# amoretti86/PSVO

Measured on AMD Instinct MI355X. Metric: particle-steps/sec, higher is better.
Workload: dtype f32

## Files before the change

psvo_amd/csrc/bsim_bwd2_impl.h:

```cpp
#pragma once
#define PSVO_BSIM_BWD_V2_UNIT 1
#include "bsim_bwd_impl.h"

namespace psvo {
PSVO_TIMERS_DEFINE(bsim_bwd2)

#define PSVO_GARG(args_type, field) ::psvo::as_global(PSVO_ARG(args_type, field))

__device__ __forceinline__ float swap_add32(float lo, float hi) {
    asm volatile("s_nop 1\n\tv_permlane32_swap_b32 %0, %1" : "+v"(lo), "+v"(hi));
    return lo + hi;
}
__device__ __forceinline__ float swap_add16(float lo, float hi) {
    asm volatile("s_nop 1\n\tv_permlane16_swap_b32 %0, %1" : "+v"(lo), "+v"(hi));
    return lo + hi;
}
__device__ __forceinline__ float row_sum16(float v) {
    v += dpp_mov<0x128, 0xF, 0xF, true>(v, v);
    v += dpp_mov<0x124, 0xF, 0xF, true>(v, v);
    v += dpp_mov<0x122, 0xF, 0xF, true>(v, v);
    v += dpp_mov<0x121, 0xF, 0xF, true>(v, v);
    return v;
}

__device__ __forceinline__ float rs_bit3(float lo, float hi) {
    float r;
    asm volatile("s_nop 1\n\t"
                 "v_add_f32_dpp %0, %1, %1 row_ror:8 row_mask:0xf bank_mask:0x3\n\t"
                 "v_add_f32_dpp %0, %2, %2 row_ror:8 row_mask:0xf bank_mask:0xc"
                 : "=&v"(r) : "v"(lo), "v"(hi));
    return r;
}
__device__ __forceinline__ float rs_bit2(float lo, float hi) {
    float r;
    asm volatile("s_nop 1\n\t"
                 "v_add_f32_dpp %0, %1, %1 row_shl:4 row_mask:0xf bank_mask:0x5\n\t"
                 "v_add_f32_dpp %0, %2, %2 row_shr:4 row_mask:0xf bank_mask:0xa"
                 : "=&v"(r) : "v"(lo), "v"(hi));
    return r;
}
template <int K>
__device__ __forceinline__ void row_reduce_scatter(const float (&v)[4 * K], float (&out)[K]) {
    float h[2 * K];
#pragma unroll
    for (int i = 0; i < 2 * K; ++i) h[i] = rs_bit3(v[i], v[2 * K + i]);
#pragma unroll
    for (int i = 0; i < K; ++i) out[i] = group_sum<4>(rs_bit2(h[i], h[K + i]));
}

typedef float f4v __attribute__((ext_vector_type(4)));
typedef __bf16 bf8v __attribute__((ext_vector_type(8)));

__device__ __forceinline__ void bf16_split3(float v, unsigned& h, unsigned& m, unsigned& l) {
    const unsigned hb = __float_as_uint(v) & 0xffff0000u;
    const float r = v - __uint_as_float(hb);
    const unsigned mb = __float_as_uint(r) & 0xffff0000u;
    const float r2 = r - __uint_as_float(mb);
    h = hb >> 16;
    m = mb >> 16;
    l = __float_as_uint(r2) >> 16;
}
__device__ __forceinline__ uint4 bf16x3_a(float v) {
    unsigned h, m, l;
    bf16_split3(v, h, m, l);
    return make_uint4(h | (h << 16), m | (h << 16), l | (m << 16), m | (l << 16));
}
__device__ __forceinline__ uint4 bf16x3_b(float v) {
    unsigned h, m, l;
    bf16_split3(v, h, m, l);
    return make_uint4(h | (m << 16), h | (l << 16), h | (m << 16), l | (m << 16));
}

template <int DX, int DY, int H, int M, int JM>
__global__ void __launch_bounds__(256, 2) bsim_bwd2_kernel(const BsimBwdArgs a) {
    using MQ = MlpLds<DX, H, DX, 1>;
    using MG = MlpLds<DX, H, DY, 1>;
    using AC = BAcc<DX>;
    constexpr int kN = AC::kSg + DY;
    constexpr int PS = (JM == 3) ? 20 : (DX == 4 && JM == 0) ? 5 : BTileSlot<DX>::kFloats;
    constexpr int FO = (JM == 3) ? 16 : 0;
    constexpr int NA = DX + 1;
    constexpr int PART = 2;
    constexpr int G = M * PART;
    constexpr int CPW = 64 / G;
    constexpr int CM = CPW * M;
    constexpr int NF = DX + 2;
    constexpr int UVS = (2 * DX + 3) & ~3;
    constexpr int JC = (JM == 0 && DX == 4) ? 2 : (JM || DX >= 3) ? 4 : 8;
    constexpr bool RO = (DX == 4) && (JM == 0);
    constexpr bool kSplitTile = (DX == 4) && (JM == 0);
    static_assert(CM == 32 && (M % 4) == 0, "two lanes per (chain, m): M in {4, 8, 16, 32}");
    extern __shared__ __attribute__((aligned(16))) float smem[];

    const int tid = threadIdx.x, lane = tid & 63, wave = tid >> 6;
    constexpr int NTB = 256, nwv = 4;
    const int B = a.B, T = a.T, N = a.N;
    const int NP = ((N + 127) / 128) * 128;
    const int nch = NP / (16 * JC);
    const int b = blockIdx.y, blk = blockIdx.x, nblk = gridDim.x;
    constexpr int cpb = nwv * CPW;
    const int cl = lane / G, part = (lane / M) & 1, m = lane % M;
    const bool h0 = (part == 0);
    const int n_raw = blk * cpb + wave * CPW + cl;
    const bool valid = n_raw < N;
    const int n = valid ? n_raw : N - 1;
    const bool srow = valid && h0;
    const bool lead = srow && (m == 0);
    const int j16 = lane & 15, g = lane >> 4;

    float* wf = smem;
    float* wg = wf + MQ::kSize;
    float* wqi = wg + MG::kSize;
    float* tile = wqi + MQ::kSize;
    float* jacc = tile + 2 * NP * PS;
    float* xch = jacc + nwv * NA * NP;
    float* uvx = xch + nwv * NF * CM;
    float* red = uvx + nwv * CM * UVS;
    float* const xw = xch + wave * NF * CM;
    float* const uw = uvx + wave * CM * UVS;
    float* const ja = jacc + wave * NA * NP;

    MQ::load(wf, a.f, tid, NTB);
    MG::load(wg, a.g, tid, NTB);
    MQ::load(wqi, a.q1inv, tid, NTB);

    const float kappa = sqrtf(0.5f * kLog2e);
    float isf[DX], rp[DX], isfk[DX], isg[DY];
#pragma unroll
    for (int d = 0; d < DX; ++d) {
        isf[d] = 1.f / a.sig_f[d];
        rp[d] = isf[d] * kappa;
        isfk[d] = isf[d] / kappa;
    }
    float ikap2 = 1.f / (kappa * kappa);
#pragma unroll
    for (int e = 0; e < DY; ++e) isg[e] = 1.f / a.sig_g[e];
    float pc[DX], pic[DX], pi1[DX], pi2[DX];
#pragma unroll
    for (int d = 0; d < DX; ++d) {
        pi1[d] = 1.f / a.sig_q1inv[d];
        pi2[d] = 1.f / a.sig_bq2[d];
        pic[d] = pi1[d] + pi2[d];
        pc[d] = 1.f / pic[d];
    }
    float s_init[DX], is_init[DX], i_isig[DX], im[DX], mi[DX];
#pragma unroll
    for (int d = 0; d < DX; ++d) {
        s_init[d] = a.sig_init[d];
        is_init[d] = 1.f / s_init[d];
        i_isig[d] = 1.f / a.isig[d];
        im[d] = a.imean[b * DX + d];
        mi[d] = a.minit[b * DX + d];
    }
    if constexpr (DX <= 2) {
        keep_in_vgpr(isf); keep_in_vgpr(rp); keep_in_vgpr(isfk); keep_in_vgpr(isg); keep_in_vgpr(ikap2);
        keep_in_vgpr(pc); keep_in_vgpr(pic); keep_in_vgpr(pi1); keep_in_vgpr(pi2);
    }
    const float ninf = -__builtin_huge_valf();
    const float aw = valid ? as_global(a.dscore)[(size_t)b * N + n] : 0.f;

    const unsigned NM = (unsigned)N * M;
    unsigned o_nm = 4u * ((unsigned)b * NM + n * M + m);
    unsigned o_dnm[DX], o_knm[DY], o_dn[DX];
#pragma unroll
    for (int d = 0; d < DX; ++d) {
        o_dnm[d] = 4u * (((unsigned)b * DX + d) * NM + n * M + m);
        o_dn[d] = 4u * (((unsigned)b * DX + d) * N + n);
    }
#pragma unroll
    for (int k = 0; k < DY; ++k) o_knm[k] = 4u * (((unsigned)b * DY + k) * NM + n * M + m);
    unsigned o_n = 4u * ((unsigned)b * N + n);
    unsigned o_d = 4u * ((unsigned)b * DX), o_k = 4u * ((unsigned)b * DY);
    const unsigned s_nm = 4u * B * NM, s_dnm = s_nm * DX, s_knm = s_nm * DY, s_dn = 4u * B * DX * N, s_n = 4u * B * N,
                   s_d = 4u * B * DX, s_k = 4u * B * DY;

    float st[DX + 1], st_l = 0.f;
    int st_t = 0;
    auto put_slot = [&](float* buf, int j, const float (&raw)[DX + 1], float l) {
        float F[DX];
#pragma unroll
        for (int d = 0; d < DX; ++d) F[d] = raw[d] * rp[d];
        const float W = j < N ? (raw[DX] - l) * kLog2e : ninf;
        if constexpr (JM == 3) {
            const float Wf = fmaxf(W, -1e30f);
            uint4* q = reinterpret_cast<uint4*>(buf + j * PS);
            q[0] = bf16x3_b(F[0]);
            q[1] = bf16x3_b(F[DX > 1 ? 1 : 0]);
            q[2] = bf16x3_b(Wf - (F[0] * F[0] + F[DX > 1 ? 1 : 0] * F[DX > 1 ? 1 : 0]));
            q[3] = bf16x3_b(1.f);
            *reinterpret_cast<float4*>(buf + j * PS + 16) = make_float4(F[0], F[DX > 1 ? 1 : 0], 0.f, 0.f);
        } else if constexpr (JM == 2) {
            *reinterpret_cast<float4*>(buf + j * PS) = make_float4(F[0], F[1], W - (F[0] * F[0] + F[DX > 1 ? 1 : 0] * F[DX > 1 ? 1 : 0]), 1.f);
        } else if constexpr (DX <= 3) {
            float4 v;
            v.x = F[0];
            v.y = DX > 1 ? F[DX > 1 ? 1 : 0] : 0.f;
            v.z = DX > 2 ? F[DX > 2 ? 2 : 0] : 0.f;
            v.w = W;
            *reinterpret_cast<float4*>(buf + j * PS) = v;
        } else if constexpr (kSplitTile) {
            *reinterpret_cast<float4*>(buf + 4 * j) = make_float4(F[0], F[1], F[2], F[3]);
            buf[4 * NP + j] = W;
        } else {
            *reinterpret_cast<float4*>(buf + j * PS) = make_float4(F[0], F[1], F[2], F[3]);
            *reinterpret_cast<float4*>(buf + j * PS + 4) = make_float4(W, 0.f, 0.f, 0.f);
        }
    };
    auto tile_entry = [&](const float* buf, int j, float (&F)[DX], float& W) {
        if constexpr (kSplitTile) {
            const float4 e = *reinterpret_cast<const float4*>(buf + 4 * j);
            F[0] = e.x; F[DX > 1 ? 1 : 0] = e.y; F[DX > 2 ? 2 : 0] = e.z; F[DX > 3 ? 3 : 0] = e.w;
            W = buf[4 * NP + j];
        } else {
            read_slot<DX>(buf + j * PS, F, W);
        }
    };
    static_assert(offsetof(BsimBwdArgs, logW) - offsetof(BsimBwdArgs, Fm) == 8 &&
                  offsetof(BsimBwdArgs, lse) - offsetof(BsimBwdArgs, Fm) == 16 && offsetof(BsimBwdArgs, Fm) % 32 == 0,
                  "BsimBwdArgs: forward-tile pointer block");
    auto get_slot = [&](int tt, int j, float (&raw)[DX + 1], gptr<const float> Fm, gptr<const float> logW) {
        const unsigned tb = (unsigned)tt * B + b;
        const unsigned jc = j < N ? j : N - 1;
#pragma unroll
        for (int d = 0; d < DX; ++d) raw[d] = ldf(Fm, 4u * ((tb * DX + d) * N + jc));
        raw[DX] = ldf(logW, 4u * (tb * N + jc));
    };
    float st2[DX + 1];
    const bool two_slots = (DX >= 3) && NP > NTB;
    auto stage_load = [&](int tt) {
        unsigned long long pt[4];
        arg_block<4>((unsigned)offsetof(BsimBwdArgs, Fm), pt);
        st_t = tt;
        const gptr<const float> p_Fm = as_global<const float>(pt[0]), p_logW = as_global<const float>(pt[1]);
        st_l = ldf(as_global<const float>(pt[2]), 4u * ((unsigned)tt * B + b));
        if (tid < NP) get_slot(tt, tid, st, p_Fm, p_logW);
        if (two_slots && tid + NTB < NP) get_slot(tt, tid + NTB, st2, p_Fm, p_logW);
    };
    auto stage_store = [&](float* buf) {
        if (tid < NP) put_slot(buf, tid, st, st_l);
        if (two_slots && tid + NTB < NP) put_slot(buf, tid + NTB, st2, st_l);
        for (int j = tid + (two_slots ? 2 : 1) * NTB; j < NP; j += NTB) {
            float raw[DX + 1];
            get_slot(st_t, j, raw, PSVO_GARG(BsimBwdArgs, Fm), PSVO_GARG(BsimBwdArgs, logW));
            put_slot(buf, j, raw, st_l);
        }
    };
    if (T >= 2) {
        stage_load(0);
        stage_store(tile);
    }
    __syncthreads();

    constexpr bool kAccLds = (DX >= 3);
    constexpr int kRowsA = 2 * DX + DY, kRowsB = 5 * DX, kSlotsB = 8;
    float acc[kAccLds ? 1 : kN];
    float* const accA = red + 16 + wave * (kRowsA * 32 + kRowsB * kSlotsB);
    float* const accB = accA + kRowsA * 32;
    auto acc_is_lead = [](int k) { return k < 4 * DX || (k >= 5 * DX && k < 6 * DX); };
    auto acc_row = [](int k) {
        return k < 4 * DX ? k : k < 5 * DX ? k - 4 * DX : k < 6 * DX ? 4 * DX + (k - 5 * DX)
               : k < 7 * DX ? DX + (k - 6 * DX) : 2 * DX + (k - 7 * DX);
    };
    const int s32 = cl * M + m;
    if constexpr (kAccLds) {
        for (int i = lane; i < kRowsA * 32 + kRowsB * kSlotsB; i += 64) accA[i] = 0.f;
    } else {
#pragma unroll
        for (int i = 0; i < kN; ++i) acc[i] = 0.f;
    }
    auto acc_add = [&](int k, float v) {
        if constexpr (kAccLds) {
            if (acc_is_lead(k)) atomicAdd(&accB[acc_row(k) * kSlotsB + cl], v);
            else atomicAdd(&accA[acc_row(k) * 32 + s32], v);
        } else {
            acc[k] += v;
        }
    };
    float dX[DX];
#pragma unroll
    for (int d = 0; d < DX; ++d) dX[d] = 0.f;

    struct StepIn {
        float eps[DX], bm[DX], xp[DX], mu1[DX], y[DY], om, lam2;
        int sel;
    };
    static_assert(offsetof(BsimBwdArgs, dscore) - offsetof(BsimBwdArgs, obs) == 56 && offsetof(BsimBwdArgs, obs) % 64 == 0 &&
                  offsetof(BsimBwdArgs, eps_b) - offsetof(BsimBwdArgs, obs) == 8 &&
                  offsetof(BsimBwdArgs, bwX) - offsetof(BsimBwdArgs, obs) == 16 &&
                  offsetof(BsimBwdArgs, sel) - offsetof(BsimBwdArgs, obs) == 24 &&
                  offsetof(BsimBwdArgs, lam2_all) - offsetof(BsimBwdArgs, obs) == 32 &&
                  offsetof(BsimBwdArgs, om_all) - offsetof(BsimBwdArgs, obs) == 40 &&
                  offsetof(BsimBwdArgs, mu1_all) - offsetof(BsimBwdArgs, obs) == 48, "BsimBwdArgs: input pointer block");
    auto load_step = [&](bool lst, bool fst, StepIn& s) {
        unsigned long long pb[8];
        arg_block<8>((unsigned)offsetof(BsimBwdArgs, obs), pb);
        const gptr<const float> p_obs = as_global<const float>(pb[0]);
        const gptr<const float> p_eps = as_global<const float>(pb[1]);
        const gptr<const float> p_bwX = as_global<const float>(pb[2]);
        const gptr<const int32_t> p_sel = as_global<const int32_t>(pb[3]);
        const gptr<const float> p_lam2 = as_global<const float>(pb[4]);
        const gptr<const float> p_om = as_global<const float>(pb[5]);
        const gptr<const float> p_mu1 = as_global<const float>(pb[6]);
        const gptr<const float> p_bm = PSVO_GARG(BsimBwdArgs, bmu2);
        s.sel = ldi(p_sel, o_n);
#pragma unroll
        for (int d = 0; d < DX; ++d) {
            s.eps[d] = ldf(p_eps, o_dnm[d]);
            s.bm[d] = ldf(p_bm, o_d + 4u * d);
            s.xp[d] = lst ? 0.f : ldf(p_bwX, o_dn[d] + s_dn);
            s.mu1[d] = lst ? 0.f : ldf(p_mu1, o_dn[d]);
        }
#pragma unroll
        for (int k = 0; k < DY; ++k) s.y[k] = ldf(p_obs, o_k + 4u * k);
        s.om = ldf(p_om, o_nm);
        s.lam2 = fst ? 0.f : ldf(p_lam2, o_nm);
    };
    auto advance = [&]() {
        o_nm += s_nm; o_n += s_n; o_d += s_d; o_k += s_k;
#pragma unroll
        for (int d = 0; d < DX; ++d) { o_dnm[d] += s_dnm; o_dn[d] += s_dn; }
#pragma unroll
        for (int k = 0; k < DY; ++k) o_knm[k] += s_knm;
    };
    auto settle = [&](StepIn& s) {
        keep_in_vgpr(s.eps); keep_in_vgpr(s.bm); keep_in_vgpr(s.xp); keep_in_vgpr(s.mu1); keep_in_vgpr(s.y);
        keep_in_vgpr(s.om); keep_in_vgpr(s.lam2);
        asm volatile("" : "+v"(s.sel));
    };
    StepIn cur_in;
    load_step(T == 1, true, cur_in);
    settle(cur_in);

    phase_skew(a.skew);
    SEC_INIT(bsim_bwd2)
    for (int t = 0; t < T; ++t) {
        SEC(0);
        const bool first = (t == 0), last = (t == T - 1);
        const float* cur = tile + ((t + 1) & 1) * NP * PS;
        float* nxt = tile + (t & 1) * NP * PS;
        constexpr bool kLateTile = (DX == 4);
        if (!kLateTile && t + 1 < T && t >= 1) stage_load(t);
        advance();
        constexpr bool kLatePrefetch = (DX >= 3);
        StepIn nxt_in;
        auto prefetch = [&]() {
            if (t + 1 < T) load_step(t + 2 == T, false, nxt_in);
            else nxt_in = StepIn{};
        };
        if (!kLatePrefetch) prefetch();
        SEC(1);

        float xp[DX], eps[DX], bm[DX], mu1[DX], mu[DX], x[DX], y[DY];
        const int sel = cur_in.sel;
#pragma unroll
        for (int d = 0; d < DX; ++d) {
            eps[d] = cur_in.eps[d];
            bm[d] = cur_in.bm[d];
            xp[d] = cur_in.xp[d];
            mu1[d] = cur_in.mu1[d];
            if (!last) {
                mu[d] = pc[d] * fmaf(pi1[d], mu1[d], pi2[d] * bm[d]);
                x[d] = fmaf(pc[d], eps[d], mu[d]);
            } else {
                mu[d] = mi[d];
                x[d] = fmaf(s_init[d], eps[d], mu[d]);
            }
        }
#pragma unroll
        for (int k = 0; k < DY; ++k) y[k] = cur_in.y[k];
        const float pi_m = valid ? exp2_fast(cur_in.om * kLog2e) : 0.f;
        const float issel = (m == sel) ? 1.f : 0.f;
        const float dphi = aw * pi_m;
        const float dlam = -aw * (issel - pi_m);

        float dxt[DX];
#pragma unroll
        for (int d = 0; d < DX; ++d) dxt[d] = h0 ? issel * dX[d] : 0.f;

        SEC(2);
        if (!first) {
            if (h0) {
#pragma unroll
                for (int d = 0; d < DX; ++d) xw[d * CM + cl * M + m] = x[d] * rp[d];
                xw[DX * CM + cl * M + m] = cur_in.lam2;
                xw[(DX + 1) * CM + cl * M + m] = dlam;
            }
            __builtin_amdgcn_fence(__ATOMIC_RELEASE, "wavefront");
            __builtin_amdgcn_wave_barrier();
            __builtin_amdgcn_fence(__ATOMIC_ACQUIRE, "wavefront");

            if constexpr (RO) {
#pragma unroll 1
                for (int r = 0; r < 2; ++r) {
                    const int it4 = 4 * (4 * r + g);
                    f2 xa[DX], xb[DX], Ua[DX], Ub[DX], Va[DX], Vb[DX];
#pragma unroll
                    for (int d = 0; d < DX; ++d) {
                        const float4 v = *reinterpret_cast<const float4*>(xw + d * CM + it4);
                        xa[d] = f2{v.x, v.y};
                        xb[d] = f2{v.z, v.w};
                        Ua[d] = Ub[d] = Va[d] = Vb[d] = f2{0.f, 0.f};
                    }
                    const float4 lq = *reinterpret_cast<const float4*>(xw + DX * CM + it4);
                    const float4 dl = *reinterpret_cast<const float4*>(xw + (DX + 1) * CM + it4);
                    const f2 lqa = f2{lq.x, lq.y}, lqb = f2{lq.z, lq.w};
                    const f2 dla = f2{dl.x, dl.y}, dlb = f2{dl.z, dl.w};
#pragma unroll 1
                    for (int c = 0; c < nch; ++c) {
                        float A2[JC][NA];
#pragma unroll
                        for (int jt = 0; jt < JC; ++jt) {
                            float F[DX], W;
                            tile_entry(cur, (c * JC + jt) * 16 + j16, F, W);
                            f2 ua[DX], ub[DX], la = f2{W, W}, lb = la;
#pragma unroll
                            for (int d = 0; d < DX; ++d) {
                                const f2 Fd = f2{F[d], F[d]};
                                ua[d] = xa[d] - Fd;
                                ub[d] = xb[d] - Fd;
                                la = pk_fma(-ua[d], ua[d], la);
                                lb = pk_fma(-ub[d], ub[d], lb);
                            }
                            la -= lqa;
                            lb -= lqb;
                            const f2 pa = f2{exp2_fast(la.x), exp2_fast(la.y)}, pb = f2{exp2_fast(lb.x), exp2_fast(lb.y)};
                            const f2 ca = dla * pa, cb = dlb * pb;
#pragma unroll
                            for (int d = 0; d < DX; ++d) {
                                const f2 pua = pa * ua[d], pub = pb * ub[d];
                                Ua[d] += pua;
                                Ub[d] += pub;
                                Va[d] = pk_fma(pua, ua[d], Va[d]);
                                Vb[d] = pk_fma(pub, ub[d], Vb[d]);
                            }
                            const f2 cs = ca + cb;
                            A2[jt][DX] = cs.x + cs.y;
#pragma unroll
                            for (int d = 0; d < DX; ++d) {
                                const f2 ad = pk_fma(cb, ub[d], ca * ua[d]);
                                A2[jt][d] = ad.x + ad.y;
                            }
                        }
                        static_assert(JC == 2, "rounds-outer flush: two tiles per chunk");
#pragma unroll
                        for (int e = 0; e < NA; ++e) {
                            float v = swap_add32(A2[0][e], A2[1][e]);
                            v += xor_lane<16>(v);
                            if ((g & 1) == 0) {
                                float* dst = ja + e * NP + (c * JC + (g >> 1)) * 16 + j16;
                                *dst = (r == 0) ? v : *dst + v;
                            }
                        }
                    }
                    float vv[4 * 2 * DX], o[UVS];
#pragma unroll
                    for (int d = 0; d < DX; ++d) {
                        vv[0 * 2 * DX + d] = Ua[d].x; vv[1 * 2 * DX + d] = Ua[d].y;
                        vv[2 * 2 * DX + d] = Ub[d].x; vv[3 * 2 * DX + d] = Ub[d].y;
                        vv[0 * 2 * DX + DX + d] = Va[d].x; vv[1 * 2 * DX + DX + d] = Va[d].y;
                        vv[2 * 2 * DX + DX + d] = Vb[d].x; vv[3 * 2 * DX + DX + d] = Vb[d].y;
                    }
                    float red2[2 * DX];
                    row_reduce_scatter<2 * DX>(vv, red2);
#pragma unroll
                    for (int e = 0; e < UVS; ++e) o[e] = e < 2 * DX ? red2[e < 2 * DX ? e : 0] : 0.f;
                    if ((j16 & 3) == 0) {
                        float* dst = uw + (4 * (4 * r + g) + (j16 >> 2)) * UVS;
#pragma unroll
                        for (int e = 0; e < UVS; e += 4)
                            *reinterpret_cast<float4*>(dst + e) = make_float4(o[e], o[e + 1], o[e + 2], o[e + 3]);
                    }
                }
            } else {
            f2 Ua[2][DX], Ub[2][DX], Va[2][DX], Vb[2][DX];
#pragma unroll
            for (int r = 0; r < 2; ++r)
#pragma unroll
                for (int d = 0; d < DX; ++d) Ua[r][d] = Ub[r][d] = Va[r][d] = Vb[r][d] = f2{0.f, 0.f};

            for (int c = 0; c < nch; ++c) {
                float A2[JC][NA];
                f4v D4[JC];
#pragma unroll
                for (int jt = 0; jt < JC; ++jt) {
#pragma unroll
                    for (int e = 0; e < NA; ++e) A2[jt][e] = 0.f;
                    D4[jt] = f4v{0.f, 0.f, 0.f, 0.f};
                }
                const float* cbase = cur + (c * 16 * JC + j16) * PS;
#pragma unroll
                for (int r = 0; r < 2; ++r) {
                    const int it4 = 4 * (4 * r + g);
                    f2 xa[DX], xb[DX];
#pragma unroll
                    for (int d = 0; d < DX; ++d) {
                        const float4 v = *reinterpret_cast<const float4*>(xw + d * CM + it4);
                        xa[d] = f2{v.x, v.y};
                        xb[d] = f2{v.z, v.w};
                    }
                    const float4 lq = *reinterpret_cast<const float4*>(xw + DX * CM + it4);
                    const float4 dl = *reinterpret_cast<const float4*>(xw + (DX + 1) * CM + it4);
                    const f2 lqa = f2{lq.x, lq.y}, lqb = f2{lq.z, lq.w};
                    const f2 dla = f2{dl.x, dl.y}, dlb = f2{dl.z, dl.w};
                    float xop[4];
                    if constexpr (JM == 1) {
#pragma unroll
                        for (int rr = 0; rr < 4; ++rr) {
                            float v = (j16 == DX) ? 1.f : 0.f;
#pragma unroll
                            for (int d = 0; d < DX; ++d) {
                                const float xv = (rr == 0) ? xa[d].x : (rr == 1) ? xa[d].y : (rr == 2) ? xb[d].x : xb[d].y;
                                v = (j16 == d) ? xv : v;
                            }
                            xop[rr] = v;
                        }
                    }
                    float sop = 0.f;
                    uint4 aop = make_uint4(0u, 0u, 0u, 0u);
                    if constexpr (JM >= 2) {
                        const int sl = 16 * r + j16;
                        const float x0 = xw[sl], x1 = xw[CM + sl], l2 = xw[DX * CM + sl];
                        sop = (g == 0) ? 2.f * x0 : (g == 1) ? 2.f * x1 : (g == 2) ? 1.f : -fmaf(x0, x0, fmaf(x1, x1, l2));
                        if constexpr (JM == 3) aop = bf16x3_a(sop);
                    }
                    if constexpr (JM >= 2) {
                        auto exponents = [&](const float* sp) -> f4v {
                            if constexpr (JM == 2) {
                                return __builtin_amdgcn_mfma_f32_16x16x4f32(sop, sp[g], f4v{0.f, 0.f, 0.f, 0.f}, 0, 0, 0);
                            } else {
                                const uint4 bq = *reinterpret_cast<const uint4*>(sp + 4 * g);
                                return __builtin_amdgcn_mfma_f32_16x16x32_bf16(__builtin_bit_cast(bf8v, aop),
                                                                               __builtin_bit_cast(bf8v, bq),
                                                                               f4v{0.f, 0.f, 0.f, 0.f}, 0, 0, 0);
                            }
                        };
                        f4v Sn = exponents(cbase);
#pragma unroll
                        for (int jt = 0; jt < JC; ++jt) {
                            const float* sp = cbase + jt * 16 * PS;
                            const float2 F2 = *reinterpret_cast<const float2*>(sp + FO);
                            const f4v S = Sn;
                            if (jt + 1 < JC) Sn = exponents(sp + 16 * PS);
                            const f2 pa = f2{exp2_fast(S[0]), exp2_fast(S[1])}, pb = f2{exp2_fast(S[2]), exp2_fast(S[3])};
                            const f2 ca = dla * pa, cb = dlb * pb;
                            const f2 Fv = f2{F2.x, F2.y}, Fq = Fv * Fv;
                            Ua[r][0] = pk_fma(pa, f2{Fv.x, Fv.x}, Ua[r][0]);
                            Ub[r][0] = pk_fma(pb, f2{Fv.x, Fv.x}, Ub[r][0]);
                            Ua[r][DX > 1 ? 1 : 0] = pk_fma(pa, f2{Fv.y, Fv.y}, Ua[r][DX > 1 ? 1 : 0]);
                            Ub[r][DX > 1 ? 1 : 0] = pk_fma(pb, f2{Fv.y, Fv.y}, Ub[r][DX > 1 ? 1 : 0]);
                            Va[r][0] = pk_fma(pa, f2{Fq.x, Fq.x}, Va[r][0]);
                            Vb[r][0] = pk_fma(pb, f2{Fq.x, Fq.x}, Vb[r][0]);
                            Va[r][DX > 1 ? 1 : 0] = pk_fma(pa, f2{Fq.y, Fq.y}, Va[r][DX > 1 ? 1 : 0]);
                            Vb[r][DX > 1 ? 1 : 0] = pk_fma(pb, f2{Fq.y, Fq.y}, Vb[r][DX > 1 ? 1 : 0]);
                            const f2 cs = ca + cb;
                            A2[jt][DX] += cs.x + cs.y;
#pragma unroll
                            for (int d = 0; d < DX; ++d) {
                                const f2 ad = pk_fma(cb, xb[d], ca * xa[d]);
                                A2[jt][d] += ad.x + ad.y;
                            }
                        }
                    } else
#pragma unroll
                    for (int jt = 0; jt < JC; ++jt) {
                        float F[DX], W;
                        if constexpr (kSplitTile) tile_entry(cur, (c * JC + jt) * 16 + j16, F, W);
                        else read_slot<DX>(cbase + jt * 16 * PS, F, W);
                        f2 ua[DX], ub[DX], la = f2{W, W}, lb = la;
#pragma unroll
                        for (int d = 0; d < DX; ++d) {
                            const f2 Fd = f2{F[d], F[d]};
                            ua[d] = xa[d] - Fd;
                            ub[d] = xb[d] - Fd;
                            la = pk_fma(-ua[d], ua[d], la);
                            lb = pk_fma(-ub[d], ub[d], lb);
                        }
                        la -= lqa;
                        lb -= lqb;
                        const f2 pa = f2{exp2_fast(la.x), exp2_fast(la.y)}, pb = f2{exp2_fast(lb.x), exp2_fast(lb.y)};
                        const f2 ca = dla * pa, cb = dlb * pb;
#pragma unroll
                        for (int d = 0; d < DX; ++d) {
                            const f2 pua = pa * ua[d], pub = pb * ub[d];
                            Ua[r][d] += pua;
                            Ub[r][d] += pub;
                            Va[r][d] = pk_fma(pua, ua[d], Va[r][d]);
                            Vb[r][d] = pk_fma(pub, ub[d], Vb[r][d]);
                        }
                        if constexpr (JM != 1) {
                            const f2 cs = ca + cb;
                            A2[jt][DX] += cs.x + cs.y;
#pragma unroll
                            for (int d = 0; d < DX; ++d) {
                                const f2 ad = pk_fma(cb, ub[d], ca * ua[d]);
                                A2[jt][d] += ad.x + ad.y;
                            }
                        } else {
                            D4[jt] = __builtin_amdgcn_mfma_f32_16x16x4f32(xop[0], ca.x, D4[jt], 0, 0, 0);
                            D4[jt] = __builtin_amdgcn_mfma_f32_16x16x4f32(xop[1], ca.y, D4[jt], 0, 0, 0);
                            D4[jt] = __builtin_amdgcn_mfma_f32_16x16x4f32(xop[2], cb.x, D4[jt], 0, 0, 0);
                            D4[jt] = __builtin_amdgcn_mfma_f32_16x16x4f32(xop[3], cb.y, D4[jt], 0, 0, 0);
                        }
                    }
                }
                if constexpr (JM != 1) {
                    float v[JC][NA];
#pragma unroll
                    for (int jt = 0; jt < JC; ++jt)
#pragma unroll
                        for (int e = 0; e < NA; ++e) v[jt][e] = A2[jt][e];
#pragma unroll
                    for (int jt = 0; jt < JC / 2; ++jt)
#pragma unroll
                        for (int e = 0; e < NA; ++e) v[jt][e] = swap_add32(v[jt][e], v[jt + JC / 2][e]);
#pragma unroll
                    for (int jt = 0; jt < JC / 4; ++jt)
#pragma unroll
                        for (int e = 0; e < NA; ++e) v[jt][e] = swap_add16(v[jt][e], v[jt + JC / 4][e]);
                    const int jt0 = (JC / 2) * (g >> 1) + (JC / 4) * (g & 1);
#pragma unroll
                    for (int jt = 0; jt < JC / 4; ++jt) {
                        if constexpr (JM >= 2) {
                            const float2 F2 = *reinterpret_cast<const float2*>(cbase + (jt0 + jt) * 16 * PS + FO);
                            v[jt][0] = fmaf(-F2.x, v[jt][DX], v[jt][0]);
                            v[jt][DX > 1 ? 1 : 0] = fmaf(-F2.y, v[jt][DX], v[jt][DX > 1 ? 1 : 0]);
                        }
#pragma unroll
                        for (int e = 0; e < NA; ++e) ja[e * NP + (c * JC + jt0 + jt) * 16 + j16] = v[jt][e];
                    }
                } else {
                    if (g == 0 || DX > 3) {
#pragma unroll
                        for (int jt = 0; jt < JC; ++jt) {
                            float F[DX], W;
                            read_slot<DX>(cbase + jt * 16 * PS, F, W);
                            (void)W;
                            const int j = (c * JC + jt) * 16 + j16;
                            if constexpr (DX <= 3) {
                                const float sc = D4[jt][DX];
#pragma unroll
                                for (int d = 0; d < DX; ++d) ja[d * NP + j] = D4[jt][d] - F[d] * sc;
                                ja[DX * NP + j] = sc;
                            } else {
                                const float sc = __shfl(D4[jt][0], 16 + j16);
                                if (g == 0) {
#pragma unroll
                                    for (int d = 0; d < DX; ++d) ja[d * NP + j] = D4[jt][d] - F[d] * sc;
                                    ja[DX * NP + j] = sc;
                                }
                            }
                        }
                    }
                }
            }
#pragma unroll
            for (int r = 0; r < 2; ++r) {
                float vv[4 * 2 * DX], o[UVS];
#pragma unroll
                for (int d = 0; d < DX; ++d) {
                    vv[0 * 2 * DX + d] = Ua[r][d].x; vv[1 * 2 * DX + d] = Ua[r][d].y;
                    vv[2 * 2 * DX + d] = Ub[r][d].x; vv[3 * 2 * DX + d] = Ub[r][d].y;
                    vv[0 * 2 * DX + DX + d] = Va[r][d].x; vv[1 * 2 * DX + DX + d] = Va[r][d].y;
                    vv[2 * 2 * DX + DX + d] = Vb[r][d].x; vv[3 * 2 * DX + DX + d] = Vb[r][d].y;
                }
                float red2[2 * DX];
                row_reduce_scatter<2 * DX>(vv, red2);
#pragma unroll
                for (int e = 0; e < UVS; ++e) o[e] = e < 2 * DX ? red2[e < 2 * DX ? e : 0] : 0.f;
                if ((j16 & 3) == 0) {
                    float* dst = uw + (4 * (4 * r + g) + (j16 >> 2)) * UVS;
#pragma unroll
                    for (int e = 0; e < UVS; e += 4)
                        *reinterpret_cast<float4*>(dst + e) = make_float4(o[e], o[e + 1], o[e + 2], o[e + 3]);
                }
            }
            }
            __builtin_amdgcn_fence(__ATOMIC_RELEASE, "wavefront");
            __builtin_amdgcn_wave_barrier();
            __builtin_amdgcn_fence(__ATOMIC_ACQUIRE, "wavefront");
            SEC(3);
            if (h0) {
                float uv[UVS];
#pragma unroll
                for (int e = 0; e < UVS; e += 4) {
                    const float4 q4 = *reinterpret_cast<const float4*>(uw + (cl * M + m) * UVS + e);
                    uv[e] = q4.x; uv[e + 1] = q4.y; uv[e + 2] = q4.z; uv[e + 3] = q4.w;
                }
                if constexpr (JM >= 2) {
#pragma unroll
                    for (int d = 0; d < DX; ++d) {
                        const float xs = x[d] * rp[d], r1 = uv[d], r2 = uv[DX + d];
                        uv[d] = xs - r1;
                        uv[DX + d] = fmaf(xs, xs - 2.f * r1, r2);
                    }
                }
#pragma unroll
                for (int d = 0; d < DX; ++d) {
                    dxt[d] -= dlam * uv[d] * isfk[d];
                    acc_add(AC::kSf + d, dlam * (uv[DX + d] * ikap2 - 1.f) * isf[d]);
                }
            }
        } else {
#pragma unroll
            for (int d = 0; d < DX; ++d) {
                const float z = (x[d] - im[d]) * i_isig[d];
                const float tz = dphi * z * i_isig[d];
                if (h0) {
                    dxt[d] -= tz;
                    acc_add(AC::kSiota + d, dphi * (z * z - 1.f) * i_isig[d]);
                }
            }
        }

        if (kLatePrefetch) prefetch();
        if (kLateTile && t + 1 < T && t >= 1) stage_load(t);
        SEC(4);
        float dxp_part[DX];
#pragma unroll
        for (int d = 0; d < DX; ++d) dxp_part[d] = 0.f;
        {
            float dFo[DX];
#pragma unroll
            for (int d = 0; d < DX; ++d) dFo[d] = 0.f;
            if (!last) {
                float fmx[DX];
                MQ::template eval_part<PART>(wf, part, x, fmx);
#pragma unroll
                for (int d = 0; d < DX; ++d) fmx[d] += xor_lane<M>(fmx[d]);
#pragma unroll
                for (int d = 0; d < DX; ++d) {
                    const float z = (xp[d] - fmx[d]) * isf[d];
                    dFo[d] = dphi * z * isf[d];
                    if (h0) {
                        dxp_part[d] = -dFo[d];
                        acc_add(AC::kSf + d, dphi * (z * z - 1.f) * isf[d]);
                    }
                }
                MQ::template bwd_input_part<PART>(wf, part, x, dFo, dxt);
            }
            static_assert(offsetof(BsimBwdArgs, dFt) - offsetof(BsimBwdArgs, xt) == 8 &&
                          offsetof(BsimBwdArgs, dGt) - offsetof(BsimBwdArgs, xt) == 16 &&
                          offsetof(BsimBwdArgs, dmu1) - offsetof(BsimBwdArgs, xt) == 24 && offsetof(BsimBwdArgs, xt) % 32 == 0,
                          "BsimBwdArgs: row pointer block");
            unsigned long long pr[4];
            arg_block<4>((unsigned)offsetof(BsimBwdArgs, xt), pr);
            if (srow) {
#pragma unroll
                for (int d = 0; d < DX; ++d) {
                    stf(as_global<float>(pr[1]), o_dnm[d] - s_dnm, dFo[d]);
                    stf(as_global<float>(pr[0]), o_dnm[d] - s_dnm, x[d]);
                }
            }
            float gm[DY], dGo[DY];
            MG::template eval_part<PART>(wg, part, x, gm);
#pragma unroll
            for (int k = 0; k < DY; ++k) gm[k] += xor_lane<M>(gm[k]);
#pragma unroll
            for (int k = 0; k < DY; ++k) {
                float dmean = 1.f;
                if (a.emission) { dmean = emis_dmean(gm[k]); gm[k] = emis_mean(gm[k]); }
                const float z = (y[k] - gm[k]) * isg[k];
                dGo[k] = dphi * z * isg[k] * dmean;
                if (h0) acc_add(AC::kSg + k, dphi * (z * z - 1.f) * isg[k]);
                if (srow) stf(as_global<float>(pr[2]), o_knm[k] - s_knm, dGo[k]);
            }
            MG::template bwd_input_part<PART>(wg, part, x, dGo, dxt);
        }

        SEC(5);
        float dmu[DX], sce[DX], dxp[DX], dim[DX];
#pragma unroll
        for (int d = 0; d < DX; ++d) {
            const float v3 = (first && h0) ? dphi * (x[d] - im[d]) * i_isig[d] * i_isig[d] : 0.f;
            dmu[d] = group_sum<G>(dxt[d]);
            sce[d] = group_sum<G>(dxt[d] * eps[d]);
            dxp[d] = group_sum<G>(dxp_part[d]);
            dim[d] = first ? group_sum<G>(v3) : 0.f;
        }
        float outv[DX];
        if (!last) {
            float dmu1[DX];
#pragma unroll
            for (int d = 0; d < DX; ++d) {
                dmu1[d] = dmu[d] * pc[d] * pi1[d];
                outv[d] = dmu[d] * pc[d] * pi2[d];
                if (lead) {
                    stf(PSVO_GARG(BsimBwdArgs, dmu1), o_dn[d] - s_dn, dmu1[d]);
                    acc_add(AC::kSc + d, sce[d] + aw * pic[d]);
                    acc_add(AC::kSmm1 + d, dmu[d] * mu1[d]);
                    acc_add(AC::kSmb + d, dmu[d] * bm[d]);
                    acc_add(AC::kSmm + d, dmu[d] * mu[d]);
                }
            }
            {
                constexpr int kQS = (H / 4 < G) ? H / 4 : G;
                float dq[DX];
#pragma unroll
                for (int d = 0; d < DX; ++d) dq[d] = 0.f;
                MQ::template bwd_input_part<kQS>(wqi, (lane % G) & (kQS - 1), xp, dmu1, dq);
#pragma unroll
                for (int d = 0; d < DX; ++d) dxp[d] += group_sum<kQS>(dq[d]);
            }
        } else {
#pragma unroll
            for (int d = 0; d < DX; ++d) {
                outv[d] = dmu[d];
                if (lead) {
                    stf(PSVO_GARG(BsimBwdArgs, dmu1), o_dn[d] - s_dn, 0.f);
                    acc_add(AC::kSinit + d, sce[d] + aw * is_init[d]);
                }
            }
        }
#pragma unroll
        for (int d = 0; d < DX; ++d) dX[d] = dxp[d];
        if (lead) {
#pragma unroll
            for (int d = 0; d < DX; ++d) {
                stf(PSVO_GARG(BsimBwdArgs, dbmu2_rows), o_dn[d] - s_dn, last ? 0.f : outv[d]);
                if (last) PSVO_GARG(BsimBwdArgs, dminit_rows)[((size_t)b * DX + d) * N + n] = outv[d];
                if (first) PSVO_GARG(BsimBwdArgs, dimean_rows)[((size_t)b * DX + d) * N + n] = dim[d];
            }
        }
        SEC(6);
        __syncthreads();
        settle(nxt_in);
        cur_in = nxt_in;
        const size_t tb = (size_t)t * B + b;
        if (!first) {
            const size_t tbm = tb - B;
            const gptr<float> pF = PSVO_GARG(BsimBwdArgs, dFm_part) + (tbm * nblk + blk) * DX * N;
            const gptr<float> pW = PSVO_GARG(BsimBwdArgs, dlogW_part) + (tbm * nblk + blk) * N;
            for (int j = tid; j < N; j += NTB) {
#pragma unroll
                for (int d = 0; d < NA; ++d) {
                    const float* col = jacc + d * NP + j;
                    const float a0 = col[0], a1 = col[NA * NP], a2 = col[2 * NA * NP], a3 = col[3 * NA * NP];
                    const float s = (a0 + a1) + (a2 + a3);
                    if (d < DX) pF[d * N + j] = s * isfk[d < DX ? d : 0];
                    else pW[j] = s;
                }
            }
        }
        if (last) {
            const gptr<float> pF = PSVO_GARG(BsimBwdArgs, dFm_part) + (tb * nblk + blk) * DX * N;
            const gptr<float> pW = PSVO_GARG(BsimBwdArgs, dlogW_part) + (tb * nblk + blk) * N;
            for (int j = tid; j < N; j += NTB) {
#pragma unroll
                for (int d = 0; d < DX; ++d) pF[d * N + j] = 0.f;
                pW[j] = 0.f;
            }
        }
        SEC(7);
        if (t + 1 < T && t >= 1) stage_store(nxt);
        __syncthreads();
        SEC(8);
    }

    for (int i = 0; i < kN; ++i) {
        float v = 0.f;
        if constexpr (kAccLds) {
            if (acc_is_lead(i)) v = lane < kSlotsB ? accB[acc_row(i) * kSlotsB + lane] : 0.f;
            else v = lane < 32 ? accA[acc_row(i) * 32 + lane] : 0.f;
        } else {
#pragma unroll
            for (int k = 0; k < kN; ++k) v = (k == i) ? acc[k] : v;
        }
        v = wave_sum(v);
        if (lane == 0) red[wave] = v;
        __syncthreads();
        if (tid == 0) {
            float s = 0.f;
            for (int w = 0; w < nwv; ++w) s += red[w];
            as_global(a.sacc_part)[((size_t)b * nblk + blk) * kN + i] = s;
        }
        __syncthreads();
    }
}

static inline void bsim2_geometry(int N, int M, int& cpb, int& nblk) {
    cpb = 4 * (64 / (2 * M));
    nblk = (N + cpb - 1) / cpb;
}

static inline bool bsim2_supported(int B, int T, int N, int M, int Dx, int Dy) {
    if (pick_m(M, [](auto) { return PSVO_OK; }) != PSVO_OK) return false;
    const long long big = (long long)T * B * (Dx > Dy ? Dx : Dy) * N * M * 4;
    return big < (1ll << 32);
}

template <int DX, int DY, int H, int M>
static int launch_bsim_bwd2(const BsimBwdArgs& a, const BsimBwdOut& o, int jm, hipStream_t stream) {
    using MQ = MlpLds<DX, H, DX, 1>;
    using MG = MlpLds<DX, H, DY, 1>;
    const int PS = (jm == 3 && DX == 2) ? 20 : (DX == 4) ? 5 : BTileSlot<DX>::kFloats;
    constexpr int UVS = (2 * DX + 3) & ~3;
    int cpb, nblk;
    bsim2_geometry(a.N, M, cpb, nblk);
    const int NP = ((a.N + 127) / 128) * 128;
    const size_t lds = sizeof(float) * (2 * MQ::kSize + MG::kSize + 2 * (size_t)NP * PS + 4 * (size_t)(DX + 1) * NP +
                                        4 * (DX + 2) * 32 + 4 * 32 * UVS + 16 +
                                        (DX >= 3 ? 4 * ((2 * DX + DY) * 32 + 5 * DX * 8) : 0));
    if (lds > 160 * 1024) return PSVO_ERR_UNSUPPORTED;
    BsimBwdArgs as = a;
    as.skew = (int)(2560.0 * NP / 128.0 * (3 * DX + 4) / 10.0 * g_tune_skew_pct / 100.0);
    clear_hip_error();
    if (jm == 3 && DX == 2) {
        if constexpr (DX == 2)
            hipLaunchKernelGGL((bsim_bwd2_kernel<DX, DY, H, M, 3>), dim3(nblk, a.B), dim3(256), lds, stream, as);
    } else if (jm == 2 && DX == 2) {
        if constexpr (DX == 2)
            hipLaunchKernelGGL((bsim_bwd2_kernel<DX, DY, H, M, 2>), dim3(nblk, a.B), dim3(256), lds, stream, as);
    } else if (jm == 1 && DX == 2) {
        if constexpr (DX == 2)
            hipLaunchKernelGGL((bsim_bwd2_kernel<DX, DY, H, M, 1>), dim3(nblk, a.B), dim3(256), lds, stream, as);
    } else {
        hipLaunchKernelGGL((bsim_bwd2_kernel<DX, DY, H, M, 0>), dim3(nblk, a.B), dim3(256), lds, stream, as);
    }
    (void)o;
    return launch_status();
}

template <int DX>
int bb2_dispatch_dy(const BsimBwdArgs& a, const BsimBwdOut& o, int Dy, int H, int M, int jm, hipStream_t s) {
    return dispatch_dy_h_m(Dy, H, M, [&](auto dy, auto h, auto m) __attribute__((visibility("hidden"))) {
        return launch_bsim_bwd2<DX, dy(), h(), m()>(a, o, jm, s); });
}

}
```

Before: 258.6 million.

## Move per-step offsets into scalar bases and use DPP/permlane reductions

Per-step address advancement in vector registers is replaced by scalar row-base pointers computed from the timestep, so the per-lane offsets stay constant. Butterfly group sums switch to DPP and permlane-swap instructions instead of generic xor shuffles. Accumulator zeroing is folded into the first add, and partial-result stores go through scalar-base buffer stores. The aim is fewer VALU ops and VGPRs in the hot loop, at the cost of more inline asm and tighter coupling to gfx950 instructions.

After: 262.7 million (median of 6 runs). 1.6% higher.

```diff
diff --git a/psvo_amd/csrc/bsim_bwd2_impl.h b/psvo_amd/csrc/bsim_bwd2_impl.h
--- a/psvo_amd/csrc/bsim_bwd2_impl.h
+++ b/psvo_amd/csrc/bsim_bwd2_impl.h
@@ -39,13 +39,45 @@
                  : "=&v"(r) : "v"(lo), "v"(hi));
     return r;
 }
+template <int MASK>
+__device__ __forceinline__ float add_xor(float v) {
+    if constexpr (MASK == 4) {
+        float r;
+        asm("s_nop 1\n\t"
+            "v_add_f32_dpp %0, %1, %1 row_shl:4 row_mask:0xf bank_mask:0x5\n\t"
+            "v_add_f32_dpp %0, %1, %1 row_shr:4 row_mask:0xf bank_mask:0xa"
+            : "=&v"(r) : "v"(v));
+        return r;
+    } else if constexpr (MASK == 16) {
+        float w = v;
+        asm("s_nop 1\n\tv_permlane16_swap_b32 %0, %1" : "+v"(v), "+v"(w));
+        return v + w;
+    } else if constexpr (MASK == 32) {
+        float w = v;
+        asm("s_nop 1\n\tv_permlane32_swap_b32 %0, %1" : "+v"(v), "+v"(w));
+        return v + w;
+    } else {
+        return v + xor_lane<MASK>(v);
+    }
+}
+template <int G>
+__device__ __forceinline__ float group_sum2(float v) {
+    if constexpr (G > 1) v = add_xor<1>(v);
+    if constexpr (G > 2) v = add_xor<2>(v);
+    if constexpr (G > 4) v = add_xor<4>(v);
+    if constexpr (G > 8) v = add_xor<8>(v);
+    if constexpr (G > 16) v = add_xor<16>(v);
+    if constexpr (G > 32) v = add_xor<32>(v);
+    return v;
+}
+
 template <int K>
 __device__ __forceinline__ void row_reduce_scatter(const float (&v)[4 * K], float (&out)[K]) {
     float h[2 * K];
 #pragma unroll
     for (int i = 0; i < 2 * K; ++i) h[i] = rs_bit3(v[i], v[2 * K + i]);
 #pragma unroll
-    for (int i = 0; i < K; ++i) out[i] = group_sum<4>(rs_bit2(h[i], h[K + i]));
+    for (int i = 0; i < K; ++i) out[i] = group_sum2<4>(rs_bit2(h[i], h[K + i]));
 }
 
 typedef float f4v __attribute__((ext_vector_type(4)));
@@ -173,6 +205,12 @@
     unsigned o_d = 4u * ((unsigned)b * DX), o_k = 4u * ((unsigned)b * DY);
     const unsigned s_nm = 4u * B * NM, s_dnm = s_nm * DX, s_knm = s_nm * DY, s_dn = 4u * B * DX * N, s_n = 4u * B * N,
                    s_d = 4u * B * DX, s_k = 4u * B * DY;
+    auto row = [](unsigned long long p, int tt, unsigned stride) { return p + (unsigned long long)((unsigned)tt * stride); };
+    auto row_base = [](gptr<float> p) {
+        unsigned long long q = (unsigned long long)p;
+        asm volatile("" : "+s"(q));
+        return as_global<float>(q);
+    };
 
     float st[DX + 1], st_l = 0.f;
     int st_t = 0;
@@ -291,36 +329,29 @@
                   offsetof(BsimBwdArgs, lam2_all) - offsetof(BsimBwdArgs, obs) == 32 &&
                   offsetof(BsimBwdArgs, om_all) - offsetof(BsimBwdArgs, obs) == 40 &&
                   offsetof(BsimBwdArgs, mu1_all) - offsetof(BsimBwdArgs, obs) == 48, "BsimBwdArgs: input pointer block");
-    auto load_step = [&](bool lst, bool fst, StepIn& s) {
+    auto load_step = [&](int tt, bool lst, bool fst, StepIn& s) {
         unsigned long long pb[8];
         arg_block<8>((unsigned)offsetof(BsimBwdArgs, obs), pb);
-        const gptr<const float> p_obs = as_global<const float>(pb[0]);
-        const gptr<const float> p_eps = as_global<const float>(pb[1]);
-        const gptr<const float> p_bwX = as_global<const float>(pb[2]);
-        const gptr<const int32_t> p_sel = as_global<const int32_t>(pb[3]);
-        const gptr<const float> p_lam2 = as_global<const float>(pb[4]);
-        const gptr<const float> p_om = as_global<const float>(pb[5]);
-        const gptr<const float> p_mu1 = as_global<const float>(pb[6]);
-        const gptr<const float> p_bm = PSVO_GARG(BsimBwdArgs, bmu2);
+        const gptr<const float> p_obs = as_global<const float>(row(pb[0], tt, s_k));
+        const gptr<const float> p_eps = as_global<const float>(row(pb[1], tt, s_dnm));
+        const gptr<const float> p_bwX = as_global<const float>(row(pb[2], tt + 1, s_dn));
+        const gptr<const int32_t> p_sel = as_global<const int32_t>(row(pb[3], tt, s_n));
+        const gptr<const float> p_lam2 = as_global<const float>(row(pb[4], tt, s_nm));
+        const gptr<const float> p_om = as_global<const float>(row(pb[5], tt, s_nm));
+        const gptr<const float> p_mu1 = as_global<const float>(row(pb[6], tt, s_dn));
+        const gptr<const float> p_bm = as_global<const float>(row((unsigned long long)PSVO_ARG(BsimBwdArgs, bmu2), tt, s_d));
         s.sel = ldi(p_sel, o_n);
 #pragma unroll
         for (int d = 0; d < DX; ++d) {
             s.eps[d] = ldf(p_eps, o_dnm[d]);
             s.bm[d] = ldf(p_bm, o_d + 4u * d);
-            s.xp[d] = lst ? 0.f : ldf(p_bwX, o_dn[d] + s_dn);
+            s.xp[d] = lst ? 0.f : ldf(p_bwX, o_dn[d]);
             s.mu1[d] = lst ? 0.f : ldf(p_mu1, o_dn[d]);
         }
 #pragma unroll
         for (int k = 0; k < DY; ++k) s.y[k] = ldf(p_obs, o_k + 4u * k);
         s.om = ldf(p_om, o_nm);
         s.lam2 = fst ? 0.f : ldf(p_lam2, o_nm);
-    };
-    auto advance = [&]() {
-        o_nm += s_nm; o_n += s_n; o_d += s_d; o_k += s_k;
-#pragma unroll
-        for (int d = 0; d < DX; ++d) { o_dnm[d] += s_dnm; o_dn[d] += s_dn; }
-#pragma unroll
-        for (int k = 0; k < DY; ++k) o_knm[k] += s_knm;
     };
     auto settle = [&](StepIn& s) {
         keep_in_vgpr(s.eps); keep_in_vgpr(s.bm); keep_in_vgpr(s.xp); keep_in_vgpr(s.mu1); keep_in_vgpr(s.y);
@@ -328,7 +359,7 @@
         asm volatile("" : "+v"(s.sel));
     };
     StepIn cur_in;
-    load_step(T == 1, true, cur_in);
+    load_step(0, T == 1, true, cur_in);
     settle(cur_in);
 
     phase_skew(a.skew);
@@ -340,11 +371,15 @@
         float* nxt = tile + (t & 1) * NP * PS;
         constexpr bool kLateTile = (DX == 4);
         if (!kLateTile && t + 1 < T && t >= 1) stage_load(t);
-        advance();
+        asm volatile("" : "+v"(o_nm), "+v"(o_n));
+#pragma unroll
+        for (int d = 0; d < DX; ++d) asm volatile("" : "+v"(o_dnm[d]), "+v"(o_dn[d]));
+#pragma unroll
+        for (int k = 0; k < DY; ++k) asm volatile("" : "+v"(o_knm[k]));
         constexpr bool kLatePrefetch = (DX >= 3);
         StepIn nxt_in;
         auto prefetch = [&]() {
-            if (t + 1 < T) load_step(t + 2 == T, false, nxt_in);
+            if (t + 1 < T) load_step(t + 1, t + 2 == T, false, nxt_in);
             else nxt_in = StepIn{};
         };
         if (!kLatePrefetch) prefetch();
@@ -445,7 +480,7 @@
 #pragma unroll
                         for (int e = 0; e < NA; ++e) {
                             float v = swap_add32(A2[0][e], A2[1][e]);
-                            v += xor_lane<16>(v);
+                            v = add_xor<16>(v);
                             if ((g & 1) == 0) {
                                 float* dst = ja + e * NP + (c * JC + (g >> 1)) * 16 + j16;
                                 *dst = (r == 0) ? v : *dst + v;
@@ -476,17 +511,22 @@
 #pragma unroll
             for (int r = 0; r < 2; ++r)
 #pragma unroll
-                for (int d = 0; d < DX; ++d) Ua[r][d] = Ub[r][d] = Va[r][d] = Vb[r][d] = f2{0.f, 0.f};
+                for (int d = 0; d < DX; ++d) {
+                    asm("v_mov_b64 %0, 0" : "=v"(Ua[r][d]));
+                    asm("v_mov_b64 %0, 0" : "=v"(Ub[r][d]));
+                    asm("v_mov_b64 %0, 0" : "=v"(Va[r][d]));
+                    asm("v_mov_b64 %0, 0" : "=v"(Vb[r][d]));
+                }
 
             for (int c = 0; c < nch; ++c) {
                 float A2[JC][NA];
                 f4v D4[JC];
-#pragma unroll
-                for (int jt = 0; jt < JC; ++jt) {
-#pragma unroll
-                    for (int e = 0; e < NA; ++e) A2[jt][e] = 0.f;
-                    D4[jt] = f4v{0.f, 0.f, 0.f, 0.f};
-                }
+                if constexpr (JM == 1) {
+#pragma unroll
+                    for (int jt = 0; jt < JC; ++jt) D4[jt] = f4v{0.f, 0.f, 0.f, 0.f};
+                }
+                constexpr bool kSeedJ = (DX <= 2);
+                auto a2_add = [&](int r, float& acc, float v) { acc = (r == 0) ? (kSeedJ ? v : 0.f + v) : acc + v; };
                 const float* cbase = cur + (c * 16 * JC + j16) * PS;
 #pragma unroll
                 for (int r = 0; r < 2; ++r) {
@@ -553,11 +593,11 @@
                             Va[r][DX > 1 ? 1 : 0] = pk_fma(pa, f2{Fq.y, Fq.y}, Va[r][DX > 1 ? 1 : 0]);
                             Vb[r][DX > 1 ? 1 : 0] = pk_fma(pb, f2{Fq.y, Fq.y}, Vb[r][DX > 1 ? 1 : 0]);
                             const f2 cs = ca + cb;
-                            A2[jt][DX] += cs.x + cs.y;
+                            a2_add(r, A2[jt][DX], cs.x + cs.y);
 #pragma unroll
                             for (int d = 0; d < DX; ++d) {
                                 const f2 ad = pk_fma(cb, xb[d], ca * xa[d]);
-                                A2[jt][d] += ad.x + ad.y;
+                                a2_add(r, A2[jt][d], ad.x + ad.y);
                             }
                         }
                     } else
@@ -589,11 +629,11 @@
                         }
                         if constexpr (JM != 1) {
                             const f2 cs = ca + cb;
-                            A2[jt][DX] += cs.x + cs.y;
+                            a2_add(r, A2[jt][DX], cs.x + cs.y);
 #pragma unroll
                             for (int d = 0; d < DX; ++d) {
                                 const f2 ad = pk_fma(cb, ub[d], ca * ua[d]);
-                                A2[jt][d] += ad.x + ad.y;
+                                a2_add(r, A2[jt][d], ad.x + ad.y);
                             }
                         } else {
                             D4[jt] = __builtin_amdgcn_mfma_f32_16x16x4f32(xop[0], ca.x, D4[jt], 0, 0, 0);
@@ -726,7 +766,7 @@
                 float fmx[DX];
                 MQ::template eval_part<PART>(wf, part, x, fmx);
 #pragma unroll
-                for (int d = 0; d < DX; ++d) fmx[d] += xor_lane<M>(fmx[d]);
+                for (int d = 0; d < DX; ++d) fmx[d] = add_xor<M>(fmx[d]);
 #pragma unroll
                 for (int d = 0; d < DX; ++d) {
                     const float z = (xp[d] - fmx[d]) * isf[d];
@@ -747,14 +787,14 @@
             if (srow) {
 #pragma unroll
                 for (int d = 0; d < DX; ++d) {
-                    stf(as_global<float>(pr[1]), o_dnm[d] - s_dnm, dFo[d]);
-                    stf(as_global<float>(pr[0]), o_dnm[d] - s_dnm, x[d]);
+                    stf(as_global<float>(row(pr[1], t, s_dnm)), o_dnm[d], dFo[d]);
+                    stf(as_global<float>(row(pr[0], t, s_dnm)), o_dnm[d], x[d]);
                 }
             }
             float gm[DY], dGo[DY];
             MG::template eval_part<PART>(wg, part, x, gm);
 #pragma unroll
-            for (int k = 0; k < DY; ++k) gm[k] += xor_lane<M>(gm[k]);
+            for (int k = 0; k < DY; ++k) gm[k] = add_xor<M>(gm[k]);
 #pragma unroll
             for (int k = 0; k < DY; ++k) {
                 float dmean = 1.f;
@@ -762,7 +802,7 @@
                 const float z = (y[k] - gm[k]) * isg[k];
                 dGo[k] = dphi * z * isg[k] * dmean;
                 if (h0) acc_add(AC::kSg + k, dphi * (z * z - 1.f) * isg[k]);
-                if (srow) stf(as_global<float>(pr[2]), o_knm[k] - s_knm, dGo[k]);
+                if (srow) stf(as_global<float>(row(pr[2], t, s_knm)), o_knm[k], dGo[k]);
             }
             MG::template bwd_input_part<PART>(wg, part, x, dGo, dxt);
         }
@@ -772,10 +812,10 @@
 #pragma unroll
         for (int d = 0; d < DX; ++d) {
             const float v3 = (first && h0) ? dphi * (x[d] - im[d]) * i_isig[d] * i_isig[d] : 0.f;
-            dmu[d] = group_sum<G>(dxt[d]);
-            sce[d] = group_sum<G>(dxt[d] * eps[d]);
-            dxp[d] = group_sum<G>(dxp_part[d]);
-            dim[d] = first ? group_sum<G>(v3) : 0.f;
+            dmu[d] = group_sum2<G>(dxt[d]);
+            sce[d] = group_sum2<G>(dxt[d] * eps[d]);
+            dxp[d] = group_sum2<G>(dxp_part[d]);
+            dim[d] = first ? group_sum2<G>(v3) : 0.f;
         }
         float outv[DX];
         if (!last) {
@@ -785,7 +825,7 @@
                 dmu1[d] = dmu[d] * pc[d] * pi1[d];
                 outv[d] = dmu[d] * pc[d] * pi2[d];
                 if (lead) {
-                    stf(PSVO_GARG(BsimBwdArgs, dmu1), o_dn[d] - s_dn, dmu1[d]);
+                    stf(as_global<float>(row((unsigned long long)PSVO_ARG(BsimBwdArgs, dmu1), t, s_dn)), o_dn[d], dmu1[d]);
                     acc_add(AC::kSc + d, sce[d] + aw * pic[d]);
                     acc_add(AC::kSmm1 + d, dmu[d] * mu1[d]);
                     acc_add(AC::kSmb + d, dmu[d] * bm[d]);
@@ -799,14 +839,14 @@
                 for (int d = 0; d < DX; ++d) dq[d] = 0.f;
                 MQ::template bwd_input_part<kQS>(wqi, (lane % G) & (kQS - 1), xp, dmu1, dq);
 #pragma unroll
-                for (int d = 0; d < DX; ++d) dxp[d] += group_sum<kQS>(dq[d]);
+                for (int d = 0; d < DX; ++d) dxp[d] += group_sum2<kQS>(dq[d]);
             }
         } else {
 #pragma unroll
             for (int d = 0; d < DX; ++d) {
                 outv[d] = dmu[d];
                 if (lead) {
-                    stf(PSVO_GARG(BsimBwdArgs, dmu1), o_dn[d] - s_dn, 0.f);
+                    stf(as_global<float>(row((unsigned long long)PSVO_ARG(BsimBwdArgs, dmu1), t, s_dn)), o_dn[d], 0.f);
                     acc_add(AC::kSinit + d, sce[d] + aw * is_init[d]);
                 }
             }
@@ -816,9 +856,13 @@
         if (lead) {
 #pragma unroll
             for (int d = 0; d < DX; ++d) {
-                stf(PSVO_GARG(BsimBwdArgs, dbmu2_rows), o_dn[d] - s_dn, last ? 0.f : outv[d]);
-                if (last) PSVO_GARG(BsimBwdArgs, dminit_rows)[((size_t)b * DX + d) * N + n] = outv[d];
-                if (first) PSVO_GARG(BsimBwdArgs, dimean_rows)[((size_t)b * DX + d) * N + n] = dim[d];
+                stf(as_global<float>(row((unsigned long long)PSVO_ARG(BsimBwdArgs, dbmu2_rows), t, s_dn)), o_dn[d], last ? 0.f : outv[d]);
+                if (first || last) {
+                    unsigned oe = o_dn[d];
+                    asm volatile("" : "+v"(oe));
+                    if (last) stf(PSVO_GARG(BsimBwdArgs, dminit_rows), oe, outv[d]);
+                    if (first) stf(PSVO_GARG(BsimBwdArgs, dimean_rows), oe, dim[d]);
+                }
             }
         }
         SEC(6);
@@ -830,14 +874,16 @@
             const size_t tbm = tb - B;
             const gptr<float> pF = PSVO_GARG(BsimBwdArgs, dFm_part) + (tbm * nblk + blk) * DX * N;
             const gptr<float> pW = PSVO_GARG(BsimBwdArgs, dlogW_part) + (tbm * nblk + blk) * N;
+            int NPh = NP;
+            asm volatile("" : "+s"(NPh));
             for (int j = tid; j < N; j += NTB) {
 #pragma unroll
                 for (int d = 0; d < NA; ++d) {
-                    const float* col = jacc + d * NP + j;
-                    const float a0 = col[0], a1 = col[NA * NP], a2 = col[2 * NA * NP], a3 = col[3 * NA * NP];
+                    const float* col = jacc + d * NPh + j;
+                    const float a0 = col[0], a1 = col[NA * NPh], a2 = col[2 * NA * NPh], a3 = col[3 * NA * NPh];
                     const float s = (a0 + a1) + (a2 + a3);
-                    if (d < DX) pF[d * N + j] = s * isfk[d < DX ? d : 0];
-                    else pW[j] = s;
+                    if (d < DX) stf(row_base(pF + d * N), 4u * j, s * isfk[d < DX ? d : 0]);
+                    else stf(pW, 4u * j, s);
                 }
             }
         }
@@ -846,8 +892,8 @@
             const gptr<float> pW = PSVO_GARG(BsimBwdArgs, dlogW_part) + (tb * nblk + blk) * N;
             for (int j = tid; j < N; j += NTB) {
 #pragma unroll
-                for (int d = 0; d < DX; ++d) pF[d * N + j] = 0.f;
-                pW[j] = 0.f;
+                for (int d = 0; d < DX; ++d) stf(row_base(pF + d * N), 4u * j, 0.f);
+                stf(pW, 4u * j, 0.f);
             }
         }
         SEC(7);
```
